# zihang-student/Codes-of-IPD-SsN-AMG-method

Measured on AMD Instinct MI355X. Metric: V-cycle throughput (DoF*cycles/sec), m=n=1024 OT grid, higher is better.
Workload: dtype f64

## Files before the change

### codes_of_ipd_ssn_amg_method_amd/csrc/ipd_limits.h

```cpp
#pragma once

#include <cstddef>

#if defined(__HIPCC__)
#define IPD_HD_INLINE __host__ __device__ __forceinline__
#else
#define IPD_HD_INLINE inline
#endif

static constexpr int BT = 512;

static constexpr int STAGE_MAX = 7680;

static constexpr int ROW_U = 4;

static constexpr double QUEUED_NNZ_MAX = 6000.0;
static constexpr int RRC_T1_NNZ_MAX = 1 << 18;
static constexpr int PAD_ROWS_MAX = 65535;
static constexpr double PAD_AVG_MIN = 0.5;
static constexpr double PAD_SLACK_FACTOR = 1.3, PAD_SLACK = 16.0;
static constexpr int PAD_BATCHES = 8;
static constexpr int PCG_LANES_MAX = 64;

static constexpr size_t SPGEMM_LAZY_MAX = size_t(1) << 21;
static constexpr int SCAN_HEAD_MAX = 4096;
static constexpr int MIS_SMALL_ROWS = 1024;
static constexpr int MIS_SMALL_NNZ = 40000;
static constexpr double SPLIT_ROW_MIN = 256.0;
static constexpr double WIDE_ROW_MIN = 96.0;
static constexpr int SPGEMM_TILE = 64, SPGEMM_TILE_K = 16;
static constexpr size_t SPGEMM_TILE_BYTES_MAX = size_t(12) << 30;
static constexpr size_t DENSE_SCRATCH_BYTES_MAX = size_t(2) << 30;
static constexpr int SPGEMM_COLS_MAX = 16384;
static constexpr int XFER_COARSE_MAX = 8192;
static constexpr int XFER_HINT_LEVELS = 40;

static constexpr int IPD_APD_SIDE_MAX = 16384;
static constexpr int IPD_COST_DIM_MAX = 16;

static constexpr int SOLVE_ML = 24;
static constexpr size_t IMAGE_LDS_BUDGET = (size_t)150 * 1024;
static constexpr size_t IMAGE_LDS_OPTIN = (size_t)156 * 1024;
static constexpr int RELOC_MAX = 640;
static constexpr size_t SOL_HEAD = 12592;

static constexpr int PCG_SMALL_MAXIT = 1000;

static constexpr int BDENSE_Q = 24;
IPD_HD_INLINE int bdense_lanes(int N) { return N > 64 ? 4 : 8; }
IPD_HD_INLINE int bdense_pad(int N) {
    const int g = 4 * bdense_lanes(N);
    return (N + g - 1) / g * g;
}
IPD_HD_INLINE int bdense_ld(int N) {
    const int Lr = bdense_lanes(N), p = bdense_pad(N);
    return p % (2 * Lr) == Lr ? p : p + Lr;
}

static constexpr int RES_WAVES = BT / 64;
static constexpr int RES_NMAX = 4 * BT;
static constexpr int RES_P4_SEG = 128;
static constexpr int RES_TAIL_MAX = 64;
static constexpr size_t RES_LDS_BYTES = sizeof(double) * ((size_t)9 * RES_NMAX + RES_NMAX / 2 + 3 * RES_TAIL_MAX + 14 * RES_WAVES + 12 + 6 * RES_WAVES + 8);
static constexpr size_t RES_LDS_MAX = IMAGE_LDS_OPTIN;

static constexpr int RB_NMAX = 8 * BT;
static constexpr int RB_HALF = 4 * BT;
static constexpr int RB_N3MAX = 2 * BT;
static constexpr int RB_N4MAX = BT / 2;
static constexpr int RB_N5MAX = BT / 4;
static constexpr int RB_RPW_MAX = 2;
static constexpr size_t RB_LDS_DOUBLES = (size_t)2 * RB_NMAX + 3 * RB_HALF + 2 * RES_WAVES +
                                         2 * 8 * RB_RPW_MAX + 20 * 8 * RB_RPW_MAX + 8 +
                                         2 * RB_N3MAX + 2 * RB_N4MAX + RB_N5MAX + 128;
static constexpr size_t RB_LDS_BYTES = sizeof(double) * RB_LDS_DOUBLES;

static constexpr int HYBRID_N0 = 100;
static constexpr int RES_MASK_MIN_ROWS = 2048;
static constexpr size_t HYBRID_SMALL_LDS_OPTIN = (size_t)96 * 1024;
static constexpr size_t hybrid_small_lds(int nb) { return sizeof(double) * ((size_t)nb * (nb + 1) + nb); }
static_assert(hybrid_small_lds(HYBRID_N0) <= HYBRID_SMALL_LDS_OPTIN, "a small block of HYBRID_N0 rows must fit the LDS opted in to");
```

### codes_of_ipd_ssn_amg_method_amd/csrc/ipd_resident.h

```cpp
#pragma once

#include "ipd_resident_proto.h"

static constexpr int RES_P3_LD = 1152;
static constexpr int RES_P4_LD = 2 * RES_P4_SEG + 64;

struct ResLevelDesc {
    int N, nf, S;
    const unsigned short* pci;
    const double* pva;
    const double* diag;
    const double* dinv;
    const double* Axi;
    const double* xx;
};
struct ResDesc {
    ResLevelDesc L1, L2;
    ResLevelDesc L3;
    ResCsr Pt2, P2;
    ResCsr Pt3, P3;
    ResCsr Pt4, P4;
    ResCsr A3;
    ResCsr A4;
    int three;
// ... 136 lines not shown
    a = __hiloint2double((int)hi[0], (int)lo[0]);
    b = __hiloint2double((int)hi[1], (int)lo[1]);
}
__device__ __forceinline__ void res_cs_rows(const double (&A)[RES_WAVES][2], double v0, double v1, double* part_out,
                                            int w, int lane) {
    static_assert(RES_WAVES == 8, "eight rows per block and workgroup");
    double p[RES_WAVES];
#pragma unroll
    for (int r = 0; r < RES_WAVES; ++r) p[r] = __builtin_fma(A[r][1], v1, A[r][0] * v0);
    double q[4];
#pragma unroll
    for (int k = 0; k < 4; ++k) {
        res_swap_halves32(p[k], p[k + 4]);
        q[k] = p[k] + p[k + 4];
    }
    double t[2];
#pragma unroll
    for (int k = 0; k < 2; ++k) {
        res_swap_rows16(q[k], q[k + 2]);
        t[k] = q[k] + q[k + 2];
    }
    const bool f = (lane & 8) != 0;
    const double keep = f ? t[1] : t[0], send = f ? t[0] : t[1];
    double u = keep + dpp_get<0x128, 0xf>(send);
    u = subwave_sum(u, 8);
    if ((lane & 7) == 0) part_out[8 * (lane >> 3) + w] = u;
}

enum res_class {
    RES_CL_HALF = 0,
    RES_CL_START = 1,
    RES_CL_RR = 2,
    RES_CL_RESTRICT = 3,
    RES_CL_LEVEL2 = 4,
    RES_CL_PROLONG = 5,
    RES_CL_TOP = 6,
    RES_NCLASS = 8
};

template <int KE1, int KE2, int KE3 = 0, bool POLY2 = false, bool DIAG = true, bool FULL = false>
__global__ __launch_bounds__(BT, 2) void k_resident(const ResDesc D, const double* __restrict__ bvec,
                                                    double* xg, double* out, int fixed_cycles) {
    static_assert(!POLY2 || (KE3 == 0 && KE1 == 16), "POLY2: three-level hierarchies in column slices (resident_takes_poly2)");
    static_assert(!FULL || POLY2, "FULL: the composed instantiation only (resident_takes_full)");
    static_assert(DIAG || KE1 == 16, "the production form exists for the column-slice kernels");
    constexpr int FG = 2 * BT / RES_WAVES;
    if constexpr (FULL) __builtin_assume(__builtin_amdgcn_workitem_id_x() < (unsigned)BT);
    constexpr bool THREE = KE3 > 0;
    constexpr bool POLY3 = KE3 == 1;
    constexpr int K3 = (THREE && !POLY3) ? KE3 : 2;
    extern __shared__ __attribute__((aligned(16))) char res_smem[];
    double* sm = reinterpret_cast<double*>(res_smem);
    const char* smb = res_smem;
    const int tid = threadIdx.x, w = tid >> 6, lane = tid & 63;
#define RES_REMOTE (FULL ? 0 : D.remote)
#define RES_WIDENT (FULL ? 1 : D.wident)
    const int b = blockIdx.x, G = FULL ? FG : gridDim.x - (RES_REMOTE ? 1 : 0);
    const int N1 = FULL ? 4 * BT : D.L1.N, N2 = FULL ? 2 * BT : D.L2.N, nf = FULL ? 2 * BT : D.L1.nf, nc = N1 - nf;
    const int Nt = FULL ? 1 : D.Nt;
    if (RES_REMOTE && b == G) {
        __shared__ PhaseLds tail_lds;
        __shared__ double tail_red[16];
        __shared__ double tail_part[48 + SOLVE_ML + 1];
        __shared__ int tail_stat[RES_WAVES];
        res_tail_workgroup(D.tail, res_smem, &tail_lds, tail_red, tail_part, tail_stat);
        return;
    }
    constexpr int oX = 0, oE1 = RES_NMAX, oE2 = 2 * RES_NMAX, oRR1 = 3 * RES_NMAX;
    constexpr int oR1 = 4 * RES_NMAX, oAX1 = 5 * RES_NMAX, oR2 = 6 * RES_NMAX, oRR2 = 7 * RES_NMAX;
    constexpr int oAX2 = 8 * RES_NMAX;
    constexpr int oRHO = 9 * RES_NMAX;
    constexpr int oBETA = oAX2 + RES_NMAX / 2;
    constexpr int oU = oRR2;
    constexpr int oR3 = 9 * RES_NMAX + RES_NMAX / 2, oE3 = oR3 + RES_TAIL_MAX, oP3 = oE3 + RES_TAIL_MAX;
    constexpr int oPART = oR3, oPART9 = oR3 + 2 * RES_WAVES * RES_WAVES;
    static_assert(2 * RES_WAVES * RES_WAVES + 2 * RES_WAVES <= 3 * RES_TAIL_MAX, "the totals fit the tail's slots");
    constexpr int oRED = oP3 + RES_TAIL_MAX;
    constexpr int oPUB = oRED + 2 * RES_WAVES;
    constexpr int oOWN = oPUB + 2 * RES_WAVES;
    int* fail = reinterpret_cast<int*>(sm + oOWN + 10 * RES_WAVES);
    long long* dbg_acc = reinterpret_cast<long long*>(sm + oOWN + 10 * RES_WAVES + 1);
    int* rowp = reinterpret_cast<int*>(sm + oOWN + 10 * RES_WAVES + 12);
    unsigned* cls_acc = reinterpret_cast<unsigned*>(sm + oOWN + 10 * RES_WAVES + 12 + 6 * RES_WAVES);
    constexpr int oE3L = oE2 + RES_NMAX / 2, oR3L = oRR2 + RES_NMAX / 2, oRR3L = oRR2 + 3 * RES_NMAX / 4;
    constexpr int oR4L = oRR3L + 128, oE5L = oRR3L + 256, oPS4 = oRR3L + 320;
    constexpr int oAX3L = oAX2 + RES_NMAX / 2;
    const int N3 = THREE ? D.L3.N : 0;
    double* red = sm + oRED;

    const int loF = FULL ? b * RES_WAVES : (int)(((long long)b * nf) / G);
    const int hiF = FULL ? loF + RES_WAVES : (int)(((long long)(b + 1) * nf) / G);
    const int loC = FULL ? nf + b * RES_WAVES : nf + (int)(((long long)b * nc) / G);
    const int hiC = FULL ? loC + RES_WAVES : nf + (int)(((long long)(b + 1) * nc) / G);
    const int lo2 = FULL ? b * RES_WAVES : (int)(((long long)b * N2) / G);
    const int hi2 = FULL ? lo2 + RES_WAVES : (int)(((long long)(b + 1) * N2) / G);
#define RES_OWN_ROW(lo, hi, l) (FULL ? (lo) + ((l) & (RES_WAVES - 1)) : ((lo) + (l) < (hi) ? (lo) + (l) : (hi) - 1))
    const int rowF = loF + w, rowC = loC + w, row2 = lo2 + w;
    const bool vF = rowF < hiF, vC = rowC < hiC, v2 = row2 < hi2;
    const int rF = vF ? rowF : 0, rC = vC ? rowC : 0, r2 = v2 ? row2 : 0;
    const int lo3 = THREE ? (int)(((long long)b * N3) / G) : 0, hi3 = THREE ? (int)(((long long)(b + 1) * N3) / G) : 0;
    const int row3 = lo3 + w;
    const bool v3 = THREE && row3 < hi3;
    const int r3 = v3 ? row3 : 0;

    constexpr bool CS1 = KE1 == 16;
    constexpr int KR1 = CS1 ? 4 : KE1;
    unsigned cF[KR1 / 2], cC[KR1 / 2], c2[KE2 / 2];
    double aF[KR1], aC[KR1], a2[KE2];
    double AF[RES_WAVES][2], AC[RES_WAVES][2];
    (void)cF; (void)cC; (void)aF; (void)aC; (void)AF; (void)AC;
    if constexpr (CS1) {
        constexpr int SW = 2 * BT;
        bool lost = false;
#pragma unroll
        for (int blk = 0; blk < 2; ++blk) {
            for (int i = tid; i < RES_WAVES * SW; i += BT) sm[i] = 0.0;
            __syncthreads();
            const int row = blk == 0 ? rF : rC, c0 = blk == 0 ? nf : 0, ncol = blk == 0 ? nc : nf;
            if (blk == 0 ? vF : vC)
                for (int e = lane; e < D.L1.S; e += 64) {
                    const size_t off = (size_t)row * D.L1.S + e;
                    const int k = (int)D.L1.pci[off] - c0;
                    const double aa = D.L1.pva[off];
                    if (aa != 0.0) {
                        if (k >= 0 && k < ncol && k < SW)
                            sm[w * SW + k] = aa;
                        else
                            lost = true;
                    }
                }
            __syncthreads();
#pragma unroll
            for (int r = 0; r < RES_WAVES; ++r)
#pragma unroll
                for (int u = 0; u < 2; ++u) {
                    const double aa = sm[r * SW + tid + u * BT];
                    if (blk == 0) AF[r][u] = aa; else AC[r][u] = aa;
                }
            __syncthreads();
        }
        if (lost) {
            __hip_atomic_store(D.tmo + 1, 1u, __ATOMIC_RELAXED, __HIP_MEMORY_SCOPE_AGENT);
            __hip_atomic_store(D.tmo, 0x7ffffffeu, __ATOMIC_RELEASE, __HIP_MEMORY_SCOPE_AGENT);
        }
    } else {
        res_load_slice<KR1>(D.L1, rF, vF, lane, cF, aF);
        res_load_slice<KR1>(D.L1, rC, vC, lane, cC, aC);
    }
    double B2[RES_WAVES][2];
    (void)B2;
    if constexpr (POLY2) {
#pragma unroll
        for (int r = 0; r < RES_WAVES; ++r)
#pragma unroll
            for (int u = 0; u < 2; ++u) {
                const int col = tid + u * BT;
                const bool ok = lo2 + r < hi2 && col < N2;
                const double bv = D.p2rows[(size_t)(ok ? lo2 + r : 0) * D.p2ld + D.p2seg + (ok ? col : 0)];
                B2[r][u] = ok ? bv : 0.0;
            }
    } else {
        res_load_slice<KE2>(D.L2, r2, v2, lane, c2, a2);
    }
    unsigned c3[K3 / 2];
    double a3[K3];
    if (THREE && !POLY3) res_load_slice<K3>(D.L3, r3, v3, lane, c3, a3);
// ... 168 lines not shown
        __syncthreads();                                                                           \
        if (dbg) dbg_acc[3] += __builtin_amdgcn_s_memtime();                                       \
        if (w == 0) {                                                                              \
            const int l8_ = lane & (RES_WAVES - 1);                                                \
            const bool second_ = lane >= RES_WAVES;                                                \
            if (lane < 2 * RES_WAVES && l8_ < (second_ ? (cB) : (cA)) &&                           \
                !RES_SKIPPED(seq))                                                                 \
                res_publish(rs, seq, (second_ ? (gB) : (gA)) + l8_, (PUBV));                       \
        }                                                                                          \
        double p0 = 0.0, p1 = 0.0;                                                                 \
        _Pragma("unroll") for (int u_ = 0; u_ < NJ; ++u_) {                                        \
            const int j = tid + u_ * BT;                                                           \
            if (j < (n)) { PRE; }                                                                  \
        }                                                                                          \
        EXTRA;                                                                                     \
        if (dbg) dbg_acc[0] -= __builtin_amdgcn_s_memtime();                                       \
        for (int ps_ = 0; ps_ < D.presleep; ++ps_) __builtin_amdgcn_s_sleep(1);                    \
        if (res_sweep<NJ>(rs, seq, (n), dead, D.tmo, hv_, D.pollsleep)) {                             \
            *fail = 1;                                                                             \
            if (lane == 0) __hip_atomic_store(D.tmo, seq, __ATOMIC_RELAXED, __HIP_MEMORY_SCOPE_AGENT); \
        }                                                                                          \
        if (dbg) {                                                                                 \
            const long long t_ = __builtin_amdgcn_s_memtime();                                     \
            dbg_acc[0] += t_;                                                                      \
            dbg_acc[4] -= t_;                                                                      \
        }                                                                                          \
        _Pragma("unroll") for (int u_ = 0; u_ < NJ; ++u_) {                                        \
            const int j = tid + u_ * BT;                                                           \
            if (j < (n)) {                                                                         \
                const double v = hv_[u_];                                                          \
                STORE;                                                                             \
            }                                                                                      \
        }                                                                                          \
        AFTER;                                                                                     \
        if (want_sums) {                                                                           \
            p0 = wave_sum(p0);                                                                     \
            if ((want_sums) > 1) p1 = wave_sum(p1);                                                \
            if (lane == 0) {                                                                       \
                red[w] = p0;                                                                       \
                if ((want_sums) > 1) red[RES_WAVES + w] = p1;                                      \
            }                                                                                      \
        }                                                                                          \
        if (dbg) {                                                                                 \
            const long long t_ = __builtin_amdgcn_s_memtime();                                     \
            dbg_acc[4] += t_;                                                                      \
            dbg_acc[5] -= t_;                                                                      \
        }                                                                                          \
        __syncthreads();                                                                           \
        if (dbg) dbg_acc[5] += __builtin_amdgcn_s_memtime();                                       \
        if (want_sums) {                                                                           \
            t0 = res_red8_tree(red);                                                               \
            if ((want_sums) > 1) t1 = res_red8_tree(red + RES_WAVES);                              \
        }                                                                                          \
    } while (0)

    auto masked_sum = [&](unsigned bits, int off, int n) __attribute__((always_inline)) {
        double s0 = 0.0, s1 = 0.0;
        (void)n;
        const double* base = sm + off + lane;
        for (int q0 = 0; q0 < 16; q0 += 8) {
            double x[8];
#pragma unroll
            for (int q = 0; q < 8; ++q) x[q] = base[64 * (q0 + q)];
            const unsigned bq = bits >> q0;
#pragma unroll
            for (int q = 0; q < 8; q += 2) {
                s0 += ((bq >> q) & 1u) ? x[q] : 0.0;
                s1 += ((bq >> (q + 1)) & 1u) ? x[q + 1] : 0.0;
            }
        }
        return wave_sum(s0 + s1);
    };
    double c1 = 0.0, c2s = 0.0;
    double sumr2p = 0.0;
    (void)sumr2p;
    const double p2ws = POLY2 ? D.p2w[N2] : 0.0;
    double dum0 = 0.0, dum1 = 0.0;
    (void)dum0;
    (void)dum1;

    int csFed = -1, csBuf = 0;
    double eFo = 0.0, eCo = 0.0;
    (void)csFed; (void)csBuf; (void)eFo; (void)eCo;
    auto cs_both_rows = [&](int off) __attribute__((always_inline)) {
        const double f0 = tid < nc ? sm[off + nf + tid] : 0.0, f1 = tid + BT < nc ? sm[off + nf + tid + BT] : 0.0;
        const double g0 = tid < nf ? sm[off + tid] : 0.0, g1 = tid + BT < nf ? sm[off + tid + BT] : 0.0;
        res_cs_rows(AF, f0, f1, sm + oPART, w, lane);
        res_cs_rows(AC, g0, g1, sm + oPART + RES_WAVES * RES_WAVES, w, lane);
        csFed = -1;
        eFo = eCo = 0.0;
    };

    auto cs_row_value = [&](int off, bool rhs_b) __attribute__((always_inline)) {
        const bool sec = lane >= RES_WAVES;
        const int r = lane & (RES_WAVES - 1);
        const int row = sec ? RES_OWN_ROW(loC, hiC, r) : RES_OWN_ROW(loF, hiF, r);
        const double T = res_red8_tree(sm + oPART + RES_WAVES * lane);
        const double dg_ = sm[oOWN + (sec ? 3 : 0) * RES_WAVES + r];
        const double base = rhs_b ? sm[oOWN + (sec ? 5 : 2) * RES_WAVES + r] : sm[oR1 + row];
        return base - (T + dg_ * sm[off + row]);
    };

    auto top = [&]() __attribute__((always_inline)) {
        if constexpr (CS1) {
            cls_begin(RES_CL_TOP);
            cs_both_rows(oX);
        } else {
        const double sF = wave_sum(res_rowdot_fma<KR1, 8 * oX>(cF, aF, smb));
        const double sC = wave_sum(res_rowdot_fma<KR1, 8 * oX>(cC, aC, smb));
        if (lane == 0) {
            sm[oPUB + w] = bF - (sF + dgF * sm[oX + rF]);
            sm[oPUB + RES_WAVES + w] = bC - (sC + dgC * sm[oX + rC]);
        }
        }
        double nrm2 = 0.0, sumr = 0.0;
        if constexpr (CS1)
            RES_HANDOFF_PV(4, N1, loF, hiF - loF, loC, hiC - loC, cs_row_value(oX, true), {},
                           { sm[oR1 + j] = v; sm[oE1 + j] = 0.0; p0 += v * v; p1 += v; }, {}, 2, nrm2, sumr);
        else
        RES_HANDOFF(4, N1, loF, hiF - loF, loC, hiC - loC,
                    { sm[oR1 + j] = v; sm[oE1 + j] = 0.0; p0 += v * v; p1 += v; }, {}, 2, nrm2, sumr);
        c1 = nsp ? sumr * rxx1 : 0.0;
        if (lfirst) {
            for (int j = tid; j < nf; j += BT) {
                const double g_i = sm[oR1 + j] - sm[oAX1 + j] * c1;
                sm[oE1 + j] = sm[oDV1 + j] * g_i;
            }
            __syncthreads();
        }
        cls_end(RES_CL_TOP);
        return sqrt(nrm2);
    };

    auto cs_finish = [&](bool frows, bool first, bool zs, unsigned sq) __attribute__((always_inline)) {
        if (dbg) dbg_acc[8] -= __builtin_amdgcn_s_memtime();
        const double cc = c1;
        if (w == 0 && lane < RES_WAVES) {
            const int row = frows ? RES_OWN_ROW(loF, hiF, lane) : RES_OWN_ROW(loC, hiC, lane);
            const int g0 = frows ? loF : loC - nf, cnt = frows ? hiF - loF : hiC - loC;
            const double dg_ = sm[oOWN + (frows ? 0 : 3) * RES_WAVES + lane];
            const double dv_ = sm[oOWN + (frows ? 1 : 4) * RES_WAVES + lane];
            const double r_own = sm[oR1 + row], ax_own = sm[oAX1 + row];
            const double T = zs ? 0.0 : res_red8_tree(sm + oPART + RES_WAVES * RES_WAVES * csBuf + RES_WAVES * lane);
            const double eo = frows ? eFo : eCo;
            const double s = T + dg_ * eo;
            const double g_i = r_own - s - ax_own * cc;
            const double wv = eo + dv_ * g_i;
            if (lane < cnt && !RES_SKIPPED(sq)) res_publish(rs, sq, g0 + lane, wv);
            const double mine = first ? wv : wv + cc;
            if (frows) {
                eFo = mine;
                if (!first) eCo = eCo + cc;
            } else {
                eCo = mine;
                if (!first) eFo = eFo + cc;
            }
        }
        if (dbg) dbg_acc[8] += __builtin_amdgcn_s_memtime();
    };
    auto half1_cs = [&](bool frows, bool first, bool ezero, bool feed, bool start) __attribute__((always_inline)) {
        const int blk0 = frows ? 0 : nf, nblk = frows ? nf : nc;
        const int oth0 = frows ? nf : 0, noth = frows ? nc : nf;
        const int me = frows ? 0 : 1;
        cls_begin(start ? RES_CL_START : RES_CL_HALF);
        ++seq;
        if (*fail) dead = true;
        if (ezero && first) {
            eFo = eCo = 0.0;
            cs_finish(frows, first, true, seq);
        } else if (csFed != me) {
            const double v0 = tid < noth ? sm[oE1 + oth0 + tid] : 0.0;
            const double v1 = tid + BT < noth ? sm[oE1 + oth0 + tid + BT] : 0.0;
            csBuf ^= 1;
            if (frows)
                res_cs_rows(AF, v0, v1, sm + oPART + RES_WAVES * RES_WAVES * csBuf, w, lane);
            else
                res_cs_rows(AC, v0, v1, sm + oPART + RES_WAVES * RES_WAVES * csBuf, w, lane);
            eFo = sm[oE1 + RES_OWN_ROW(loF, hiF, lane)];
            eCo = sm[oE1 + RES_OWN_ROW(loC, hiC, lane)];
            __syncthreads();
            cs_finish(frows, first, false, seq);
        }
        const double cc = c1;
        double pa[2] = {0.0, 0.0}, pb[2] = {0.0, 0.0}, p0 = 0.0;
        if (!first) {
#pragma unroll
            for (int u = 0; u < 2; ++u) {
                const int j = tid + u * BT;
                if (j < nblk) {
                    pa[u] = sm[oR1 + blk0 + j];
                    pb[u] = sm[oAX1 + blk0 + j];
                }
            }
            for (int jo = tid; jo < noth; jo += BT) {
                const double en = sm[oE1 + oth0 + jo] + cc;
                sm[oE1 + oth0 + jo] = en;
                p0 += sm[oR1 + oth0 + jo] - sm[oAX1 + oth0 + jo] * en;
            }
        }
        if (dbg) dbg_acc[0] -= __builtin_amdgcn_s_memtime();
        for (int ps = 0; ps < D.presleep; ++ps) __builtin_amdgcn_s_sleep(1);
        double hv[2] = {0.0, 0.0};
        if (res_sweep<2>(rs, seq, nblk, dead, D.tmo, hv, D.pollsleep)) {
            *fail = 1;
            if (lane == 0) __hip_atomic_store(D.tmo, seq, __ATOMIC_RELAXED, __HIP_MEMORY_SCOPE_AGENT);
        }
        if (dbg) {
            const long long t_ = __builtin_amdgcn_s_memtime();
            dbg_acc[0] += t_;
            dbg_acc[4] -= t_;
        }
        double en[2];
#pragma unroll
        for (int u = 0; u < 2; ++u) {
            const int j = tid + u * BT;
            en[u] = j < nblk ? (first ? hv[u] : hv[u] + cc) : 0.0;
        }
        if (feed) {
            csBuf ^= 1;
            if (frows)
                res_cs_rows(AC, en[0], en[1], sm + oPART + RES_WAVES * RES_WAVES * csBuf, w, lane);
            else
                res_cs_rows(AF, en[0], en[1], sm + oPART + RES_WAVES * RES_WAVES * csBuf, w, lane);
            csFed = 1 - me;
        } else {
            csFed = -1;
        }
#pragma unroll
        for (int u = 0; u < 2; ++u) {
            const int j = tid + u * BT;
            if (j < nblk) {
                sm[oE1 + blk0 + j] = en[u];
                if (!first) p0 += pa[u] - pb[u] * en[u];
            }
        }
        double* part9 = sm + oPART9 + RES_WAVES * (int)(seq & 1);
        if (!first && nsp) {
            p0 = wave_sum(p0);
            if (lane == 0) part9[w] = p0;
        }
        if (dbg) {
            const long long t_ = __builtin_amdgcn_s_memtime();
            dbg_acc[4] += t_;
            dbg_acc[3] -= t_;
        }
        __syncthreads();
        if (dbg) dbg_acc[3] += __builtin_amdgcn_s_memtime();
        if (!first) c1 = nsp ? res_red8_tree(part9) * rxx1 : 0.0;
        if (feed)
            cs_finish(!frows, !first, false, seq + 1);
        else
            eFo = eCo = 0.0;
        cls_end(start ? RES_CL_START : RES_CL_HALF);
    };
    auto half1 = [&](bool frows, bool first, bool ezero) __attribute__((always_inline)) {
        if constexpr (!CS1) {
        double s = 0.0, eo = 0.0;
        const int row = frows ? rowF : rowC;
        const bool valid = frows ? vF : vC;
        const int rr_ = valid ? row : 0;
        if (!ezero) eo = sm[oE1 + rr_];
        const double dg_ = frows ? dgF : dgC, dv_ = frows ? dvF : dvC;
        const double r_own = sm[oR1 + rr_], ax_own = sm[oAX1 + rr_];
        if (!(ezero && first)) s = wave_sum(frows ? res_rowdot_fma<KR1, 8 * oE1>(cF, aF, smb) : res_rowdot_fma<KR1, 8 * oE1>(cC, aC, smb));
        s += dg_ * eo;
        const double g_i = r_own - s - ax_own * c1;
        const double wv = eo + dv_ * g_i;
        const int blk0 = frows ? 0 : nf, nblk = frows ? nf : nc;
        if (lane == 0) sm[oPUB + w] = wv;
        const int g0 = (frows ? loF : loC) - blk0, cnt = frows ? hiF - loF : hiC - loC;
        if (first) {
            RES_HANDOFF(2, nblk, g0, cnt, 0, 0, { sm[oE1 + blk0 + j] = v; }, {}, 0, dum0, dum1);
        } else {
            const int oth0 = frows ? nf : 0, noth = frows ? nc : nf;
            const double cc = c1;
            double xig = 0.0;
            RES_HANDOFF_P(2, nblk, g0, cnt, 0, 0,
                          { pa_[u_] = sm[oR1 + blk0 + j]; pb_[u_] = sm[oAX1 + blk0 + j]; },
                          {
                              const double en = v + cc;
                              sm[oE1 + blk0 + j] = en;
                              p0 += pa_[u_] - pb_[u_] * en;
                          },
                          {
                              for (int jo = tid; jo < noth; jo += BT) {
                                  const double en = sm[oE1 + oth0 + jo] + cc;
                                  sm[oE1 + oth0 + jo] = en;
                                  p0 += sm[oR1 + oth0 + jo] - sm[oAX1 + oth0 + jo] * en;
                              }
                          },
                          (nsp ? 1 : 0), xig, dum1);
            c1 = nsp ? xig * rxx1 : 0.0;
        }
        }
    };
    auto sweep1 = [&](bool post, bool ezero, bool last, bool start) __attribute__((always_inline)) {
        (void)start;
        if constexpr (CS1) {
            const bool local = lfirst && ezero && !post;
            if (!local) half1_cs(!post, true, ezero, true, start);
            half1_cs(post, false, ezero, !last, local);
        } else {
        if (!(lfirst && ezero && !post)) half1(!post, true, ezero);
        half1(post, false, ezero);
        }
    };

    auto sweep2 = [&](bool ezero) __attribute__((always_inline)) {
        cls_begin(RES_CL_LEVEL2);
        double s = 0.0, eo = 0.0;
        if (!ezero) {
            s = wave_sum(res_rowdot_fma<KE2, 8 * oE2>(c2, a2, smb));
            eo = sm[oE2 + r2];
            s += dg2 * eo;
        }
        const double g_i = sm[oR2 + r2] - s - sm[oAX2 + r2] * c2s;
        const double wv = eo + dv2 * g_i;
        if (lane == 0) sm[oPUB + w] = wv;
        const double cc = c2s;
        double xig = 0.0;
        RES_HANDOFF_P(4, N2, lo2, hi2 - lo2, 0, 0, { pa_[u_] = sm[oR2 + j]; pb_[u_] = sm[oAX2 + j]; },
                      {
                          const double en = v + cc;
                          sm[oE2 + j] = en;
                          p0 += pa_[u_] - pb_[u_] * en;
                      },
                      {}, (nsp ? 1 : 0), xig, dum1);
        c2s = nsp ? xig * rxx2 : 0.0;
        cls_end(RES_CL_LEVEL2);
    };

    const auto rtin = __builtin_amdgcn_make_buffer_rsrc(D.tail.tin, 0, 2 * RES_GRAN_MAX * 16, 0x00020000);
    const auto rtout = __builtin_amdgcn_make_buffer_rsrc(D.tail.tout, 0, 2 * RES_GRAN_MAX * 16, 0x00020000);
    unsigned tseq = 0;
    auto remote_tail = [&](const ResCsr& Pin, int oRRs, int oEd, int oRd, int oAXd, double xxd, int Nout,
                           double& cnext) __attribute__((always_inline)) {
        ++tseq;
        const int rin = b + G * w;
        if (rin < Nt) {
            const double s3 = res_csr_rowdot(Pin, rowp[12 * w + 6], rowp[12 * w + 7], lane, sm, oRRs);
            if (lane == 0) res_tail_post(rtin, tseq, rin, s3);
        }
        double hv[4];
        const int st = res_tail_wait<4>(rtout, tseq, Nout, D.tmo, fail, dead, lane, hv);
        double p0 = 0.0;
#pragma unroll
        for (int u = 0; u < 4; ++u) {
            const int j = tid + u * BT;
            if (j < Nout && !dead && !st) {
                const double en = sm[oEd + j] + hv[u];
                sm[oEd + j] = en;
                p0 += sm[oRd + j] - sm[oAXd + j] * en;
            }
        }
        if (nsp) {
            p0 = wave_sum(p0);
            if (lane == 0) red[w] = p0;
        }
        __syncthreads();
        if (nsp) cnext = res_red8(red) / xxd;
        if (*fail) dead = true;
    };
    auto local_tail = [&](const ResCsr& PtT, const ResCsr& AT, const ResCsr& PT, int oRRs, int oEd, int oRd,
                          int oAXd, double xxd, int Nabove, double& cnext) __attribute__((always_inline)) {
        if (Nt == 1) {
            const int e0 = PtT.rp[0], e1 = PtT.rp[1];
            double s = 0.0;
            for (int t = e0 + tid; t < e1; t += BT * 2) {
                const int t1 = t + BT;
                const int ja = PtT.ci[t], jb = PtT.ci[t1 < e1 ? t1 : e0];
                const double aa = PtT.va[t], ab = PtT.va[t1 < e1 ? t1 : e0];
                s += aa * sm[oRRs + ja];
                s += t1 < e1 ? ab * sm[oRRs + jb] : 0.0;
            }
            s = wave_sum(s);
            if (lane == 0) red[w] = s;
            __syncthreads();
            if (tid == 0) sm[oR3] = res_red8(red);
        } else {
            for (int i = w; i < Nt; i += RES_WAVES) {
                const double s = res_csr_rowdot(PtT, PtT.rp[i], PtT.rp[i + 1], lane, sm, oRRs);
                if (lane == 0) sm[oR3 + i] = s;
            }
        }
// ... 227 lines not shown
        for (int s = (lfirst2 && !keep) ? 1 : 0; s < nu; ++s) sweep2(!keep && s == 0);
        {
            cls_begin(RES_CL_LEVEL2);
            const double s = wave_sum(res_rowdot_fma<KE2, 8 * oE2>(c2, a2, smb)) + dg2 * sm[oE2 + r2];
            if (lane == 0) sm[oPUB + w] = sm[oR2 + r2] - s;
            RES_HANDOFF(4, N2, lo2, hi2 - lo2, 0, 0, { sm[oRR2 + j] = v; }, {}, 0, dum0, dum1);
        }
        if (dbg) dbg_acc[7] -= __builtin_amdgcn_s_memtime();
        if (THREE) {
            {
                const double s = res_csr_rowdot(D.Pt3, rowp[12 * w + 8], rowp[12 * w + 9], lane, sm, oRR2);
                if (lane == 0) sm[oPUB + w] = s;
                double sumr = 0.0;
                RES_HANDOFF3({ sm[oR3L + j] = v; sm[oE3L + j] = 0.0; p0 += v; }, (nsp ? 1 : 0), sumr);
                c3s = nsp ? sumr * rxx3 : 0.0;
                sumr3 = sumr;
            }
            for (int leg = 0; leg < (D.wcycle ? 2 : 1); ++leg) visit3(leg == 1);
            {
                const double sP = res_csr_rowdot(D.P3, rowp[12 * w + 10], rowp[12 * w + 11], lane, sm, oE3L);
                if (lane == 0) sm[oPUB + w] = sm[oE2 + r2] + sP;
                double xig = 0.0;
                RES_HANDOFF_P(4, N2, lo2, hi2 - lo2, 0, 0, { pa_[u_] = sm[oR2 + j]; pb_[u_] = sm[oAX2 + j]; },
                              { sm[oE2 + j] = v; p0 += pa_[u_] - pb_[u_] * v; }, {}, (nsp ? 1 : 0), xig, dum1);
                c2s = nsp ? xig * rxx2 : 0.0;
            }
        } else {
            tail();
        }
        if (dbg) dbg_acc[7] += __builtin_amdgcn_s_memtime();
        cls_end(RES_CL_LEVEL2);
        for (int s = 0; s < nu; ++s) sweep2(false);
    };

    auto poly2_fed = [&]() __attribute__((always_inline)) {
        if constexpr (POLY2) {
            ++seq;
            if (*fail) dead = true;
            if (dbg) dbg_acc[3] -= __builtin_amdgcn_s_memtime();
            __syncthreads();
            if (dbg) dbg_acc[3] += __builtin_amdgcn_s_memtime();
            const bool pub = w == 0 && lane < RES_WAVES && lane < hi2 - lo2;
            if (pub && !RES_SKIPPED(seq)) res_publish(rs, seq, lo2 + lane, sm[oPUB + lane]);
            const double s0 = tid < N2 ? sm[oP3C + tid] : 0.0, s1 = tid + BT < N2 ? sm[oP3C + tid + BT] : 0.0;
            double hv[2] = {0.0, 0.0};
            if (dbg) dbg_acc[0] -= __builtin_amdgcn_s_memtime();
            for (int ps = 0; ps < D.presleep; ++ps) __builtin_amdgcn_s_sleep(1);
            if (res_sweep<2>(rs, seq, N2, dead, D.tmo, hv, D.pollsleep)) {
                *fail = 1;
                if (lane == 0) __hip_atomic_store(D.tmo, seq, __ATOMIC_RELAXED, __HIP_MEMORY_SCOPE_AGENT);
            }
            if (dbg) {
                const long long t_ = __builtin_amdgcn_s_memtime();
                dbg_acc[0] += t_;
                dbg_acc[4] -= t_;
            }
            const double v0 = tid < N2 ? hv[0] : 0.0, v1 = tid + BT < N2 ? hv[1] : 0.0;
            res_cs_rows(B2, v0, v1, sm + oPART, w, lane);
            const double ps = wave_sum(s0 * v0 + s1 * v1);
            const double p1 = nsp ? wave_sum(v0 + v1) : 0.0;
            if (lane == 0) {
                red[w] = ps;
                red[RES_WAVES + w] = p1;
            }
            if (dbg) {
                const long long t_ = __builtin_amdgcn_s_memtime();
                dbg_acc[4] += t_;
                dbg_acc[3] -= t_;
            }
            __syncthreads();
            if (dbg) dbg_acc[3] += __builtin_amdgcn_s_memtime();
            cls_end(RES_CL_RESTRICT);
            cls_begin(RES_CL_LEVEL2);
            ++seq;
            if (*fail) dead = true;
            if (w == 0 && lane < RES_WAVES) {
                const double wB = sm[oOWN + 6 * RES_WAVES + lane], mp = sm[oOWN + 7 * RES_WAVES + lane];
                const double T = res_red8_tree(sm + oPART + RES_WAVES * lane);
                const double sr = res_red8_tree(red), sum1 = res_red8_tree(red + RES_WAVES);
                const double d = res_pcg_1x1(sr + p2ws * sum1, h33, D.pcg_maxit);
                const double val = T + wB * sum1 + mp * d;
                if (pub && !RES_SKIPPED(seq)) res_publish(rs, seq, lo2 + lane, val);
            }
            if (dbg) dbg_acc[0] -= __builtin_amdgcn_s_memtime();
            for (int ps = 0; ps < D.presleep; ++ps) __builtin_amdgcn_s_sleep(1);
            if (res_sweep<2>(rs, seq, N2, dead, D.tmo, hv, D.pollsleep)) {
                *fail = 1;
                if (lane == 0) __hip_atomic_store(D.tmo, seq, __ATOMIC_RELAXED, __HIP_MEMORY_SCOPE_AGENT);
            }
            if (dbg) {
                const long long t_ = __builtin_amdgcn_s_memtime();
                dbg_acc[0] += t_;
                dbg_acc[4] -= t_;
            }
            if (tid < N2) sm[oE2 + tid] = hv[0];
            if (tid + BT < N2) sm[oE2 + tid + BT] = hv[1];
            if (dbg) {
                const long long t_ = __builtin_amdgcn_s_memtime();
                dbg_acc[4] += t_;
                dbg_acc[5] -= t_;
            }
            __syncthreads();
            if (dbg) dbg_acc[5] += __builtin_amdgcn_s_memtime();
            cls_end(RES_CL_LEVEL2);
        }
    };

    auto cycle = [&]() __attribute__((always_inline)) {
        const int nu = D.nu;
        for (int s = 0; s < nu; ++s) sweep1(false, s == 0, s == nu - 1, s == 0);
        {
            if constexpr (CS1) {
                cls_begin(RES_CL_RR);
                cs_both_rows(oE1);
            } else {
            const double sF = wave_sum(res_rowdot_fma<KR1, 8 * oE1>(cF, aF, smb)) + dgF * sm[oE1 + rF];
            const double sC = wave_sum(res_rowdot_fma<KR1, 8 * oE1>(cC, aC, smb)) + dgC * sm[oE1 + rC];
            if (lane == 0) {
                sm[oPUB + w] = sm[oR1 + rF] - sF;
                sm[oPUB + RES_WAVES + w] = sm[oR1 + rC] - sC;
            }
            }
            if constexpr (CS1) {
                if (xm) {
                    RES_HANDOFF_PV(4, N1, loF, hiF - loF, loC, hiC - loC, cs_row_value(oE1, false),
                                   { pa_[u_] = j < nf ? sm[oRHO + j] : 1.0; },
                                   { sm[oRR1 + j] = j < nf ? v * pa_[u_] : v; }, {}, 0, dum0, dum1);
                } else {
                    RES_HANDOFF_PV(4, N1, loF, hiF - loF, loC, hiC - loC, cs_row_value(oE1, false), {},
                                   { sm[oRR1 + j] = v; }, {}, 0, dum0, dum1);
                }
            } else
            if (xm) {
                RES_HANDOFF_P(4, N1, loF, hiF - loF, loC, hiC - loC, { pa_[u_] = j < nf ? sm[oRHO + j] : 1.0; },
                              { sm[oRR1 + j] = j < nf ? v * pa_[u_] : v; }, {}, 0, dum0, dum1);
            } else {
                RES_HANDOFF(4, N1, loF, hiF - loF, loC, hiC - loC, { sm[oRR1 + j] = v; }, {}, 0, dum0, dum1);
            }
        }
        {
            cls_end(RES_CL_RR);
            cls_begin(RES_CL_RESTRICT);
            if (dbg) dbg_acc[6] -= __builtin_amdgcn_s_memtime();
            const double s = xm ? sm[oBETA + r2] * masked_sum(xbits >> 16, oRR1, nf) + sm[oRR1 + rC]
                                : res_csr_rowdot(D.Pt2, rowp[12 * w + 0], rowp[12 * w + 1], lane, sm, oRR1) +
                                      (RES_WIDENT ? sm[oRR1 + rC] : 0.0);
            if (dbg) dbg_acc[6] += __builtin_amdgcn_s_memtime();
            if (lane == 0) sm[oPUB + w] = s;
            if constexpr (POLY2) {
                poly2_fed();
            } else {
            double sumr = 0.0;
            RES_HANDOFF(4, N2, lo2, hi2 - lo2, 0, 0, { sm[oR2 + j] = v; sm[oE2 + j] = 0.0; p0 += v; }, {},
                        (nsp ? 1 : 0), sumr, dum1);
            c2s = nsp ? sumr * rxx2 : 0.0;
            sumr2p = sumr;
            if (lfirst2 && !POLY2) {
                const double cc = c2s;
                double p0 = 0.0;
                for (int j = tid; j < N2; j += BT) {
                    const double g_i = sm[oR2 + j] - sm[oAX2 + j] * cc;
                    const double en = sm[oDV2 + j] * g_i + cc;
                    sm[oE2 + j] = en;
                    p0 += sm[oR2 + j] - sm[oAX2 + j] * en;
                }
                if (nsp) {
                    p0 = wave_sum(p0);
                    if (lane == 0) red[w] = p0;
                }
                __syncthreads();
                if (nsp) c2s = res_red8(red) / xx2;
                __syncthreads();
            }
            cls_end(RES_CL_RESTRICT);
            }
        }
        if constexpr (!POLY2)
            for (int leg = 0; leg < (D.wcycle ? 2 : 1); ++leg) visit2(leg == 1);
        {
            cls_begin(RES_CL_PROLONG);
            if (dbg) dbg_acc[6] -= __builtin_amdgcn_s_memtime();
            if (xm) {
                for (int j = tid; j < N2; j += BT) sm[oU + j] = sm[oBETA + j] * sm[oE2 + j];
                __syncthreads();
            }
            const double sF = xm ? sm[oRHO + rF] * masked_sum(xbits & 0xffffu, oU, N2)
                                 : res_csr_rowdot(D.P2, rowp[12 * w + 2], rowp[12 * w + 3], lane, sm, oE2);
            const double sC = RES_WIDENT ? sm[oE2 + r2]
                                       : res_csr_rowdot(D.P2, rowp[12 * w + 4], rowp[12 * w + 5], lane, sm, oE2);
            if (dbg) dbg_acc[6] += __builtin_amdgcn_s_memtime();
            if (lane == 0) {
                sm[oPUB + w] = sm[oE1 + rF] + sF;
                sm[oPUB + RES_WAVES + w] = sm[oE1 + rC] + sC;
            }
            double xig = 0.0;
            if constexpr (CS1) {
                const bool fedpost = FULL ? true : nu >= 1 && nf <= 2 * BT;
                double fe[2] = {0.0, 0.0};
                RES_HANDOFF_PVA(4, N1, loF, hiF - loF, loC, hiC - loC, sm[oPUB + lane],
                                { pa_[u_] = sm[oR1 + j]; pb_[u_] = sm[oAX1 + j]; },
                                {
                                    sm[oE1 + j] = v;
                                    p0 += pa_[u_] - pb_[u_] * v;
                                    if (u_ < 2 && j < nf) fe[u_] = v;
                                },
                                {
                                    if (fedpost) {
                                        csBuf ^= 1;
                                        res_cs_rows(AC, fe[0], fe[1], sm + oPART + RES_WAVES * RES_WAVES * csBuf, w, lane);
                                    }
                                },
                                {}, (nsp ? 1 : 0), xig, dum1);
                c1 = nsp ? xig * rxx1 : 0.0;
                if (fedpost) {
                    eFo = sm[oE1 + RES_OWN_ROW(loF, hiF, lane)];
                    eCo = sm[oE1 + RES_OWN_ROW(loC, hiC, lane)];
                    cs_finish(false, true, false, seq + 1);
                    csFed = 1;
                }
                cls_end(RES_CL_PROLONG);
            } else {
            RES_HANDOFF_P(4, N1, loF, hiF - loF, loC, hiC - loC, { pa_[u_] = sm[oR1 + j]; pb_[u_] = sm[oAX1 + j]; },
                          { sm[oE1 + j] = v; p0 += pa_[u_] - pb_[u_] * v; }, {}, (nsp ? 1 : 0), xig, dum1);
            c1 = nsp ? xig * rxx1 : 0.0;
            }
        }
        for (int s = 0; s < nu; ++s) sweep1(true, false, s == nu - 1, s == 0 && csFed != 1);
    };

    auto add_correction = [&]() __attribute__((always_inline)) {
        for (int j = tid; j < N1; j += BT) sm[oX + j] = sm[oX + j] + sm[oE1 + j];
        __syncthreads();
    };

    const int maxit = D.maxit;
    const bool writer = b == 0 && tid == 0;
    const ResSolve sol = res_stationary(top, cycle, add_correction, D.retol, maxit, D.anycycle, fixed_cycles, dead, writer, out);
    if (RES_REMOTE && b == 0 && tid == 0)
        __hip_atomic_store(D.tail.tctl, 1u, __ATOMIC_RELAXED, __HIP_MEMORY_SCOPE_AGENT);
    if (b == 0)
        for (int j = tid; j < N1; j += BT) xg[j] = sm[oX + j];
    if (writer) {
        out[0] = (double)sol.it;
        out[1] = sol.rel_res;
        out[2] = sol.res0;
        const unsigned anytmo = __hip_atomic_load(D.tmo, __ATOMIC_ACQUIRE, __HIP_MEMORY_SCOPE_AGENT);
        out[3] = (dead || anytmo != 0) ? 1.0 : 0.0;
        if (CS1 && __hip_atomic_load(D.tmo + 1, __ATOMIC_RELAXED, __HIP_MEMORY_SCOPE_AGENT) != 0) out[3] = 2.0;
        out[4 + 2 * (maxit + 2) - 1] = (double)(seq + tseq);
    }
    if (dbg) {
        D.dbg[0] = dbg_acc[0];
        D.dbg[1] = __builtin_amdgcn_s_memtime() - dbg_acc[1];
        D.dbg[2] = seq;
        D.dbg[3] = __builtin_amdgcn_s_memrealtime() - dbg_acc[2];
        D.dbg[4] = dbg_acc[3];
        D.dbg[5] = dbg_acc[4];
        D.dbg[6] = dbg_acc[5];
        D.dbg[7] = dbg_acc[6];
        D.dbg[8] = dbg_acc[7];
        if (CS1 && !RES_REMOTE) D.dbg[9] = dbg_acc[8];
        if constexpr (CS1)
            for (int k = 0; k < 2 * RES_NCLASS; ++k) D.dbg[16 + k] = (long long)cls_acc[k];
    }
#undef RES_REMOTE
#undef RES_WIDENT
#undef RES_OWN_ROW
#undef RES_SKIPPED
#undef RES_HANDOFF3
#undef RES_HANDOFF3R
#undef RES_HANDOFF4
#undef RES_HANDOFF
#undef RES_HANDOFF_P
#undef RES_HANDOFF_PV
#undef RES_HANDOFF_PVA
#undef dgF
#undef dvF
#undef bF
#undef dgC
#undef dvC
#undef bC
#undef dg2
#undef dv2
#undef dg3
#undef dv3
}
```

Baseline: 52.33 million.

## Fuse residual publication into last half-sweep and trim barriers in FULL resident cycle

In the FULL (one wave per row, fully resident) specialization, the final smoother half-sweep now applies the coarse correction, updates x and publishes the next cycle's top residual directly. The next top step only consumes those published values, and the separate add-correction pass is skipped. A third LDS partial buffer is added so the two cs_rows products can overlap. Restriction and prolongation get specialized paths that precompute beta*e2 and merge barriers. The goal is fewer grid-wide exchange rounds and __syncthreads per V-cycle, at the cost of more LDS and extra, more intricate control-flow state (topfed) across cycles.

```diff
diff --git a/codes_of_ipd_ssn_amg_method_amd/csrc/ipd_limits.h b/codes_of_ipd_ssn_amg_method_amd/csrc/ipd_limits.h
--- a/codes_of_ipd_ssn_amg_method_amd/csrc/ipd_limits.h
+++ b/codes_of_ipd_ssn_amg_method_amd/csrc/ipd_limits.h
@@ -61,7 +61,7 @@
 static constexpr int RES_NMAX = 4 * BT;
 static constexpr int RES_P4_SEG = 128;
 static constexpr int RES_TAIL_MAX = 64;
-static constexpr size_t RES_LDS_BYTES = sizeof(double) * ((size_t)9 * RES_NMAX + RES_NMAX / 2 + 3 * RES_TAIL_MAX + 14 * RES_WAVES + 12 + 6 * RES_WAVES + 8);
+static constexpr size_t RES_LDS_BYTES = sizeof(double) * ((size_t)9 * RES_NMAX + RES_NMAX / 2 + 3 * RES_TAIL_MAX + 14 * RES_WAVES + 12 + 6 * RES_WAVES + 8 + RES_WAVES * RES_WAVES);
 static constexpr size_t RES_LDS_MAX = IMAGE_LDS_OPTIN;
 
 static constexpr int RB_NMAX = 8 * BT;
diff --git a/codes_of_ipd_ssn_amg_method_amd/csrc/ipd_resident.h b/codes_of_ipd_ssn_amg_method_amd/csrc/ipd_resident.h
--- a/codes_of_ipd_ssn_amg_method_amd/csrc/ipd_resident.h
+++ b/codes_of_ipd_ssn_amg_method_amd/csrc/ipd_resident.h
@@ -242,6 +242,8 @@
     long long* dbg_acc = reinterpret_cast<long long*>(sm + oOWN + 10 * RES_WAVES + 1);
     int* rowp = reinterpret_cast<int*>(sm + oOWN + 10 * RES_WAVES + 12);
     unsigned* cls_acc = reinterpret_cast<unsigned*>(sm + oOWN + 10 * RES_WAVES + 12 + 6 * RES_WAVES);
+    constexpr int oPART3 = oOWN + 10 * RES_WAVES + 12 + 6 * RES_WAVES + 8;
+    static_assert(!FULL || sizeof(double) * (oPART3 + RES_WAVES * RES_WAVES) <= RES_LDS_BYTES, "the third buffer lies inside the launch's LDS");
     constexpr int oE3L = oE2 + RES_NMAX / 2, oR3L = oRR2 + RES_NMAX / 2, oRR3L = oRR2 + 3 * RES_NMAX / 4;
     constexpr int oR4L = oRR3L + 128, oE5L = oRR3L + 256, oPS4 = oRR3L + 320;
     constexpr int oAX3L = oAX2 + RES_NMAX / 2;
@@ -576,6 +578,8 @@
     int csFed = -1, csBuf = 0;
     double eFo = 0.0, eCo = 0.0;
     (void)csFed; (void)csBuf; (void)eFo; (void)eCo;
+    bool topfed = false;
+    (void)topfed;
     auto cs_both_rows = [&](int off) __attribute__((always_inline)) {
         const double f0 = tid < nc ? sm[off + nf + tid] : 0.0, f1 = tid + BT < nc ? sm[off + nf + tid + BT] : 0.0;
         const double g0 = tid < nf ? sm[off + tid] : 0.0, g1 = tid + BT < nf ? sm[off + tid + BT] : 0.0;
@@ -596,6 +600,54 @@
     };
 
     auto top = [&]() __attribute__((always_inline)) {
+        double nrm2 = 0.0, sumr = 0.0;
+        bool fed = false;
+        if constexpr (FULL) {
+            if (topfed) {
+                fed = true;
+                topfed = false;
+                ++seq;
+                if (*fail) dead = true;
+                double hv[4];
+                if (dbg) dbg_acc[0] -= __builtin_amdgcn_s_memtime();
+                for (int ps = 0; ps < D.presleep; ++ps) __builtin_amdgcn_s_sleep(1);
+                if (res_sweep<4>(rs, seq, N1, dead, D.tmo, hv, D.pollsleep)) {
+                    *fail = 1;
+                    if (lane == 0) __hip_atomic_store(D.tmo, seq, __ATOMIC_RELAXED, __HIP_MEMORY_SCOPE_AGENT);
+                }
+                if (dbg) {
+                    const long long t_ = __builtin_amdgcn_s_memtime();
+                    dbg_acc[0] += t_;
+                    dbg_acc[4] -= t_;
+                }
+                double p0 = 0.0, p1 = 0.0;
+#pragma unroll
+                for (int u = 0; u < 4; ++u) {
+                    const int j = tid + u * BT;
+                    const double v = hv[u];
+                    sm[oR1 + j] = v;
+                    sm[oE1 + j] = 0.0;
+                    p0 += v * v;
+                    p1 += v;
+                }
+                p0 = wave_sum(p0);
+                p1 = wave_sum(p1);
+                if (lane == 0) {
+                    red[w] = p0;
+                    red[RES_WAVES + w] = p1;
+                }
+                if (dbg) {
+                    const long long t_ = __builtin_amdgcn_s_memtime();
+                    dbg_acc[4] += t_;
+                    dbg_acc[5] -= t_;
+                }
+                __syncthreads();
+                if (dbg) dbg_acc[5] += __builtin_amdgcn_s_memtime();
+                nrm2 = res_red8_tree(red);
+                sumr = res_red8_tree(red + RES_WAVES);
+            }
+        }
+        if (!fed) {
         if constexpr (CS1) {
             cls_begin(RES_CL_TOP);
             cs_both_rows(oX);
@@ -607,14 +659,34 @@
             sm[oPUB + RES_WAVES + w] = bC - (sC + dgC * sm[oX + rC]);
         }
         }
-        double nrm2 = 0.0, sumr = 0.0;
         if constexpr (CS1)
             RES_HANDOFF_PV(4, N1, loF, hiF - loF, loC, hiC - loC, cs_row_value(oX, true), {},
                            { sm[oR1 + j] = v; sm[oE1 + j] = 0.0; p0 += v * v; p1 += v; }, {}, 2, nrm2, sumr);
         else
         RES_HANDOFF(4, N1, loF, hiF - loF, loC, hiC - loC,
                     { sm[oR1 + j] = v; sm[oE1 + j] = 0.0; p0 += v * v; p1 += v; }, {}, 2, nrm2, sumr);
+        }
         c1 = nsp ? sumr * rxx1 : 0.0;
+        if constexpr (FULL) {
+            double e0[2];
+#pragma unroll
+            for (int u = 0; u < 2; ++u) {
+                const int j = tid + u * BT;
+                const double g_i = sm[oR1 + j] - sm[oAX1 + j] * c1;
+                e0[u] = sm[oDV1 + j] * g_i;
+                sm[oE1 + j] = e0[u];
+            }
+            csBuf ^= 1;
+            res_cs_rows(AC, e0[0], e0[1], sm + oPART + RES_WAVES * RES_WAVES * csBuf, w, lane);
+            {
+                const int row = loF + (lane & (RES_WAVES - 1));
+                const double g_i = sm[oR1 + row] - sm[oAX1 + row] * c1;
+                eFo = sm[oDV1 + row] * g_i;
+                eCo = 0.0;
+            }
+            csFed = 1;
+            __syncthreads();
+        } else
         if (lfirst) {
             for (int j = tid; j < nf; j += BT) {
                 const double g_i = sm[oR1 + j] - sm[oAX1 + j] * c1;
@@ -656,13 +728,106 @@
         const int blk0 = frows ? 0 : nf, nblk = frows ? nf : nc;
         const int oth0 = frows ? nf : 0, noth = frows ? nc : nf;
         const int me = frows ? 0 : 1;
+        if constexpr (FULL) {
+            if (!feed) {
+                cls_begin(RES_CL_HALF);
+                ++seq;
+                if (*fail) dead = true;
+                const double cc = c1;
+                double ov[2], xo[2] = {0.0, 0.0}, hv[2] = {0.0, 0.0}, mv[2];
+#pragma unroll
+                for (int u = 0; u < 2; ++u) {
+                    const int jo = oth0 + tid + u * BT;
+                    const double en = sm[oE1 + jo] + cc;
+                    sm[oE1 + jo] = en;
+                    if (frows) {
+                        const double xn = sm[oX + jo] + en;
+                        sm[oX + jo] = xn;
+                        ov[u] = xn;
+                        xo[u] = sm[oX + blk0 + tid + u * BT];
+                    } else {
+                        ov[u] = en;
+                    }
+                }
+                if (frows)
+                    res_cs_rows(AF, ov[0], ov[1], sm + oPART3, w, lane);
+                else
+                    res_cs_rows(AC, ov[0], ov[1], sm + oPART3, w, lane);
+                if (dbg) dbg_acc[0] -= __builtin_amdgcn_s_memtime();
+                for (int ps = 0; ps < D.presleep; ++ps) __builtin_amdgcn_s_sleep(1);
+                if (res_sweep<2>(rs, seq, nblk, dead, D.tmo, hv, D.pollsleep)) {
+                    *fail = 1;
+                    if (lane == 0) __hip_atomic_store(D.tmo, seq, __ATOMIC_RELAXED, __HIP_MEMORY_SCOPE_AGENT);
+                }
+                if (dbg) {
+                    const long long t_ = __builtin_amdgcn_s_memtime();
+                    dbg_acc[0] += t_;
+                    dbg_acc[4] -= t_;
+                }
+#pragma unroll
+                for (int u = 0; u < 2; ++u) {
+                    const int j = blk0 + tid + u * BT;
+                    const double en = hv[u] + cc;
+                    sm[oE1 + j] = en;
+                    if (frows) {
+                        const double xn = xo[u] + en;
+                        sm[oX + j] = xn;
+                        mv[u] = xn;
+                    } else {
+                        mv[u] = en;
+                    }
+                }
+                csBuf ^= 1;
+                if (frows)
+                    res_cs_rows(AC, mv[0], mv[1], sm + oPART + RES_WAVES * RES_WAVES * csBuf, w, lane);
+                else
+                    res_cs_rows(AF, mv[0], mv[1], sm + oPART + RES_WAVES * RES_WAVES * csBuf, w, lane);
+                if (dbg) {
+                    const long long t_ = __builtin_amdgcn_s_memtime();
+                    dbg_acc[4] += t_;
+                    dbg_acc[3] -= t_;
+                }
+                __syncthreads();
+                if (dbg) dbg_acc[3] += __builtin_amdgcn_s_memtime();
+                cls_end(RES_CL_HALF);
+                cls_begin(frows ? RES_CL_TOP : RES_CL_RR);
+                const double* totF = frows ? sm + oPART3 : sm + oPART + RES_WAVES * RES_WAVES * csBuf;
+                const double* totC = frows ? sm + oPART + RES_WAVES * RES_WAVES * csBuf : sm + oPART3;
+                if (frows) {
+                    if (w == 0 && lane < 2 * RES_WAVES) {
+                        const bool sec = lane >= RES_WAVES;
+                        const int r = lane & (RES_WAVES - 1);
+                        const int row = (sec ? loC : loF) + r;
+                        const double T = res_red8_tree((sec ? totC : totF) + RES_WAVES * r);
+                        const double dg_ = sm[oOWN + (sec ? 3 : 0) * RES_WAVES + r];
+                        const double base = sm[oOWN + (sec ? 5 : 2) * RES_WAVES + r];
+                        const double val = base - (T + dg_ * sm[oX + row]);
+                        if (!RES_SKIPPED(seq + 1)) res_publish(rs, seq + 1, row, val);
+                    }
+                    topfed = true;
+                } else {
+                    if (w == 0 && lane < RES_WAVES) {
+                        const double TF = res_red8_tree(totF + RES_WAVES * lane);
+                        const double TC = res_red8_tree(totC + RES_WAVES * lane);
+                        const double dF_ = sm[oOWN + 0 * RES_WAVES + lane], dC_ = sm[oOWN + 3 * RES_WAVES + lane];
+                        const double rF_ = sm[oR1 + loF + lane], rC_ = sm[oR1 + loC + lane];
+                        const double val = rF_ - (TF + dF_ * eFo);
+                        if (!RES_SKIPPED(seq + 1)) res_publish(rs, seq + 1, loF + lane, val);
+                        sm[oRR1 + loC + lane] = rC_ - (TC + dC_ * eCo);
+                    }
+                }
+                csFed = -1;
+                eFo = eCo = 0.0;
+                return;
+            }
+        }
         cls_begin(start ? RES_CL_START : RES_CL_HALF);
         ++seq;
         if (*fail) dead = true;
         if (ezero && first) {
             eFo = eCo = 0.0;
             cs_finish(frows, first, true, seq);
-        } else if (csFed != me) {
+        } else if (!FULL && csFed != me) {
             const double v0 = tid < noth ? sm[oE1 + oth0 + tid] : 0.0;
             const double v1 = tid + BT < noth ? sm[oE1 + oth0 + tid + BT] : 0.0;
             csBuf ^= 1;
@@ -793,7 +958,7 @@
         if constexpr (CS1) {
             const bool local = lfirst && ezero && !post;
             if (!local) half1_cs(!post, true, ezero, true, start);
-            half1_cs(post, false, ezero, !last, local);
+            half1_cs(post, false, ezero, !last, FULL ? false : local);
         } else {
         if (!(lfirst && ezero && !post)) half1(!post, true, ezero);
         half1(post, false, ezero);
@@ -1187,6 +1352,12 @@
                 const double val = T + wB * sum1 + mp * d;
                 if (pub && !RES_SKIPPED(seq)) res_publish(rs, seq, lo2 + lane, val);
             }
+            double be[2] = {0.0, 0.0};
+            (void)be;
+            if constexpr (FULL) {
+                be[0] = sm[oBETA + tid];
+                be[1] = sm[oBETA + tid + BT];
+            }
             if (dbg) dbg_acc[0] -= __builtin_amdgcn_s_memtime();
             for (int ps = 0; ps < D.presleep; ++ps) __builtin_amdgcn_s_sleep(1);
             if (res_sweep<2>(rs, seq, N2, dead, D.tmo, hv, D.pollsleep)) {
@@ -1200,6 +1371,10 @@
             }
             if (tid < N2) sm[oE2 + tid] = hv[0];
             if (tid + BT < N2) sm[oE2 + tid + BT] = hv[1];
+            if constexpr (FULL) {
+                sm[oU + tid] = be[0] * hv[0];
+                sm[oU + tid + BT] = be[1] * hv[1];
+            }
             if (dbg) {
                 const long long t_ = __builtin_amdgcn_s_memtime();
                 dbg_acc[4] += t_;
@@ -1213,7 +1388,34 @@
 
     auto cycle = [&]() __attribute__((always_inline)) {
         const int nu = D.nu;
+        if constexpr (FULL) cs_finish(false, false, false, seq + 1);
         for (int s = 0; s < nu; ++s) sweep1(false, s == 0, s == nu - 1, s == 0);
+        if constexpr (FULL) {
+            ++seq;
+            if (*fail) dead = true;
+            const double rh0 = sm[oRHO + tid], rh1 = sm[oRHO + tid + BT];
+            double hv[2] = {0.0, 0.0};
+            if (dbg) dbg_acc[0] -= __builtin_amdgcn_s_memtime();
+            for (int ps = 0; ps < D.presleep; ++ps) __builtin_amdgcn_s_sleep(1);
+            if (res_sweep<2>(rs, seq, nf, dead, D.tmo, hv, D.pollsleep)) {
+                *fail = 1;
+                if (lane == 0) __hip_atomic_store(D.tmo, seq, __ATOMIC_RELAXED, __HIP_MEMORY_SCOPE_AGENT);
+            }
+            if (dbg) {
+                const long long t_ = __builtin_amdgcn_s_memtime();
+                dbg_acc[0] += t_;
+                dbg_acc[4] -= t_;
+            }
+            sm[oRR1 + tid] = hv[0] * rh0;
+            sm[oRR1 + tid + BT] = hv[1] * rh1;
+            if (dbg) {
+                const long long t_ = __builtin_amdgcn_s_memtime();
+                dbg_acc[4] += t_;
+                dbg_acc[5] -= t_;
+            }
+            __syncthreads();
+            if (dbg) dbg_acc[5] += __builtin_amdgcn_s_memtime();
+        } else
         {
             if constexpr (CS1) {
                 cls_begin(RES_CL_RR);
@@ -1285,6 +1487,63 @@
         {
             cls_begin(RES_CL_PROLONG);
             if (dbg) dbg_acc[6] -= __builtin_amdgcn_s_memtime();
+            if constexpr (FULL) {
+                const double sF = sm[oRHO + rF] * masked_sum(xbits & 0xffffu, oU, N2);
+                if (dbg) dbg_acc[6] += __builtin_amdgcn_s_memtime();
+                if (lane == 0) sm[oPUB + w] = sm[oE1 + rF] + sF;
+                ++seq;
+                if (*fail) dead = true;
+                if (dbg) dbg_acc[3] -= __builtin_amdgcn_s_memtime();
+                __syncthreads();
+                if (dbg) dbg_acc[3] += __builtin_amdgcn_s_memtime();
+                if (w == 0 && lane < RES_WAVES && !RES_SKIPPED(seq)) res_publish(rs, seq, loF + lane, sm[oPUB + lane]);
+                double pa[2], pb[2], tc[2], hv[2] = {0.0, 0.0};
+#pragma unroll
+                for (int u = 0; u < 2; ++u) {
+                    const int j = tid + u * BT;
+                    pa[u] = sm[oR1 + j];
+                    pb[u] = sm[oAX1 + j];
+                    const double ec = sm[oE1 + nf + j] + sm[oE2 + j];
+                    sm[oE1 + nf + j] = ec;
+                    tc[u] = sm[oR1 + nf + j] - sm[oAX1 + nf + j] * ec;
+                }
+                if (dbg) dbg_acc[0] -= __builtin_amdgcn_s_memtime();
+                for (int ps = 0; ps < D.presleep; ++ps) __builtin_amdgcn_s_sleep(1);
+                if (res_sweep<2>(rs, seq, nf, dead, D.tmo, hv, D.pollsleep)) {
+                    *fail = 1;
+                    if (lane == 0) __hip_atomic_store(D.tmo, seq, __ATOMIC_RELAXED, __HIP_MEMORY_SCOPE_AGENT);
+                }
+                if (dbg) {
+                    const long long t_ = __builtin_amdgcn_s_memtime();
+                    dbg_acc[0] += t_;
+                    dbg_acc[4] -= t_;
+                }
+                double p0 = 0.0;
+#pragma unroll
+                for (int u = 0; u < 2; ++u) {
+                    sm[oE1 + tid + u * BT] = hv[u];
+                    p0 += pa[u] - pb[u] * hv[u];
+                }
+                p0 += tc[0];
+                p0 += tc[1];
+                csBuf ^= 1;
+                res_cs_rows(AC, hv[0], hv[1], sm + oPART + RES_WAVES * RES_WAVES * csBuf, w, lane);
+                p0 = wave_sum(p0);
+                if (lane == 0) red[w] = p0;
+                if (dbg) {
+                    const long long t_ = __builtin_amdgcn_s_memtime();
+                    dbg_acc[4] += t_;
+                    dbg_acc[5] -= t_;
+                }
+                __syncthreads();
+                if (dbg) dbg_acc[5] += __builtin_amdgcn_s_memtime();
+                c1 = res_red8_tree(red) * rxx1;
+                eFo = sm[oE1 + loF + (lane & (RES_WAVES - 1))];
+                eCo = sm[oE1 + loC + (lane & (RES_WAVES - 1))];
+                cs_finish(false, true, false, seq + 1);
+                csFed = 1;
+                cls_end(RES_CL_PROLONG);
+            } else {
             if (xm) {
                 for (int j = tid; j < N2; j += BT) sm[oU + j] = sm[oBETA + j] * sm[oE2 + j];
                 __syncthreads();
@@ -1329,11 +1588,15 @@
                           { sm[oE1 + j] = v; p0 += pa_[u_] - pb_[u_] * v; }, {}, (nsp ? 1 : 0), xig, dum1);
             c1 = nsp ? xig * rxx1 : 0.0;
             }
+            }
         }
         for (int s = 0; s < nu; ++s) sweep1(true, false, s == nu - 1, s == 0 && csFed != 1);
     };
 
     auto add_correction = [&]() __attribute__((always_inline)) {
+        if constexpr (FULL) {
+            if (topfed) return;
+        }
         for (int j = tid; j < N1; j += BT) sm[oX + j] = sm[oX + j] + sm[oE1 + j];
         __syncthreads();
     };
```

After: 57.70 million (median of 6 runs). 1.1x the previous value.
